# SGI-2022/Latent-Diffusion-Models-for-Shape-SDFs

Measured on AMD Instinct MI355X. Metric: SDF queries/sec on 256^3 grid (+ DDPM sample steps/sec), higher is better.
Workload: dtype bf16; 1 GPU; config4: decode B=64 shapes on a 256^3 grid on 1 rank (the whole grid is the one slab: no gather); batch=64, grid=256, latent_dim=256, decoder=DeepSDF 8x512 skip@4, parallelism=zslab1

## Files before the change

latent-diffusion-models-for-shape-sdfs_amd/csrc/decoder_fs.hip:

```cpp
#include "decoder_common.h"

namespace ldm {
namespace {
using namespace dec;

constexpr int kFsD = 4;

constexpr int kFsStep = 2048;
constexpr int kFsAct = 33 * 4 * 1024;
constexpr int kFsRed = 4 * 4 * 64 * 4;
constexpr int kFsWl = 512 * 4;
#ifndef FS_STAMP
#define FS_STAMP 0
#endif
constexpr int kFsStamp = FS_STAMP ? 128 * 8 : 0;
#ifndef FS_ABL
#define FS_ABL 0
#endif
static_assert(FS_ABL == 0 || FS_STAMP, "ablations are diagnostic builds");
constexpr int kFsLds = kFsAct + kFsRed + kFsWl + kFsStamp;
static_assert(kFsLds <= 160 * 1024, "LDS");

__host__ __device__ constexpr int fs_nparts(int S) { return S == 256 ? 15 : 16; }
__host__ __device__ constexpr int fs_nsteps(int S) { return S == 256 ? 384 : 448; }

template <typename T>
__global__ void fs_aux_pack_kernel(const float* __restrict__ beta, const float* __restrict__ wxyz,
                                   int B, T* __restrict__ aux) {
    const int id = blockIdx.x * blockDim.x + threadIdx.x;
    if (id >= B * 4 * 4 * 2 * 64) return;
    const int lane = id & 63;
    const int i = (id >> 6) & 1;
    const int slot = (id >> 7) & 3;
    const int w = (id >> 9) & 3;
    const int b = id >> 11;
    const int li = slot >> 1;
    const int p = slot & 1;
    float v[8] = {0, 0, 0, 0, 0, 0, 0, 0};
    if (lane < 32) {
        const int f = 128 * w + 64 * p + 32 * i + lane;
        const float* wx = wxyz + ((size_t)li * kHidden + f) * 3;
        const float bb = beta[((size_t)b * 2 + li) * kHidden + f];
        const float hi = Elem<T>::round(bb);
        v[0] = wx[0]; v[1] = wx[1]; v[2] = wx[2];
        v[3] = wx[0]; v[4] = wx[1]; v[5] = wx[2];
        v[6] = hi;    v[7] = bb - hi;
    }
    T* o = aux + (size_t)id * 8;
#pragma unroll
    for (int e = 0; e < 8; ++e) o[e] = (T)v[e];
}

struct FArgs {
    const uint8_t* stream;
    const uint8_t* aux;
    const float* w_last;
    const float* xyz;
    float* out;
    float b_last;
    int npts, tiles_per_shape, n_tiles;
    int N, k0;
    float vs, origin;
    const int32_t* bricks;
    const int32_t* count;
    int nb, nbt;
    GridDiv gd;
};

enum FsEpi { FE_NONE = 0, FE_LATE = 1, FE_EARLY = 2, FE_FIN0 = 3, FE_FIN1 = 4 };

struct FSrc {
    bool shape;
    uint32_t off;
    bool none = false;
};

struct FCtx {
    int lane, wave, h;
    uint32_t voff;
    char* smem;
    __amdgpu_buffer_rsrc_t rw;
    __amdgpu_buffer_rsrc_t ra;
    uint32_t s_beg, s_end;
    uint32_t s_iss;
    uint32_t baux_w;
    uint32_t aux_w;
    uint32_t aux_next;
    u32x4 auxn[2];
    u32x4 ring[kFsD][2];
    u32x4 b[4];
    float part[4];
    const f32x4* wlp;
    f32x4 wl[2][4];
    float* out;
    int npts, prev_shape, prev_local;
    float b_last;
    unsigned long long* st;
    int st_i;
    bool st_on;
    const int32_t* bricks;
    int N, nb, nbt;
};

__device__ __forceinline__ void stamp(FCtx& c) {
    if (FS_STAMP) {
        if (c.st_on && c.lane == 0 && c.st_i < 128) c.st[c.st_i] = __builtin_readcyclecounter();
        ++c.st_i;
    }
}

__device__ __forceinline__ u32x4 bld(__amdgpu_buffer_rsrc_t r, uint32_t voff, uint32_t soff) {
    return __builtin_bit_cast(u32x4, __builtin_amdgcn_raw_buffer_load_b128(r, voff, soff, 0));
}

__device__ __forceinline__ void load_aux(FCtx& c, FSrc s) {
    if (s.none) return;
    const __amdgpu_buffer_rsrc_t r = s.shape ? c.ra : c.rw;
    c.auxn[0] = bld(r, c.voff, s.off);
    c.auxn[1] = bld(r, c.voff + 1024u, s.off);
}

__device__ __forceinline__ uint32_t opaque(uint32_t v) {
    asm volatile("" : "+v"(v));
    return v;
}

__device__ __forceinline__ int opaque_s(int v) {
    asm volatile("" : "+s"(v));
    return v;
}

__device__ __forceinline__ char* lds_at(const FCtx& c, uint32_t off) {
    return c.smem + (opaque(c.voff) + off);
}
__device__ __forceinline__ char* lds_base(const FCtx& c, uint32_t off) {
    return c.smem + opaque(opaque(c.voff) + off);
}
__device__ __forceinline__ u32x4* act_wb(const FCtx& c, int late) {
    return reinterpret_cast<u32x4*>(lds_base(c, (uint32_t)(late + 4 * c.wave) * 4096u));
}
__device__ __forceinline__ u32x4* act_w(const FCtx& c, int late) {
    return reinterpret_cast<u32x4*>(lds_at(c, (uint32_t)(late + 4 * c.wave) * 4096u));
}
__device__ __forceinline__ const f32x4* wl_at(const FCtx& c, int p, int i) {
    const uint32_t h = opaque(c.voff) >> 9;
    return reinterpret_cast<const f32x4*>(
        c.smem + kFsAct + kFsRed + (((c.wave * 2 + p) * 2 + i) * 2) * 64 + h * 64);
}

__device__ __forceinline__ float* red_w(const FCtx& c) {
    return reinterpret_cast<float*>(c.smem + kFsAct + c.wave * 4 * 64 * 4 + (opaque(c.voff) >> 2));
}

__device__ __forceinline__ void fs_bar() {
    if (FS_ABL & 4) return;
    asm volatile("s_waitcnt lgkmcnt(0)\n\ts_barrier" ::: "memory");
}

__device__ __forceinline__ void read_b(FCtx& c, int pos) {
    const u32x4* p = reinterpret_cast<const u32x4*>(lds_at(c, pos * 4096));
#pragma unroll
    for (int n = 0; n < 4; ++n) c.b[n] = p[n * 64];
}

__device__ __forceinline__ void issue(FCtx& c, int r) {
    const uint32_t so = c.s_iss + (uint32_t)(r >> 1) * 2u * kFsStep;
    const uint32_t vo = c.voff + (uint32_t)(r & 1) * kFsStep;
    if (FS_ABL & 1) return;
    c.ring[r][0] = bld(c.rw, vo, so);
    c.ring[r][1] = bld(c.rw, vo + 1024u, so);
}

__device__ __forceinline__ uint32_t next_iss(const FCtx& c) {
    const uint32_t n = c.s_iss + 4u * kFsStep;
    return n == c.s_end ? c.s_beg : n;
}
__device__ __forceinline__ void next_group(FCtx& c) { c.s_iss = next_iss(c); }

__device__ __forceinline__ float relu_f(float x) {
    return __builtin_bit_cast(float, max(__builtin_bit_cast(int, x), 0));
}

__device__ __forceinline__ float acc_read(float a) {
    asm volatile("" : "+a"(a));
    return a;
}

__device__ __forceinline__ void fin1_unit(FCtx& c, const f32x16 (&accY)[2][4], int u) {
    const int t = u >> 1, s = u & 1;
    const int i = t >> 2, n = t & 3;
    const f32x4* w = wl_at(c, 1, i);
    float part = c.part[n];
#pragma unroll
    for (int q = 2 * s; q < 2 * s + 2; ++q) {
        const f32x4 wv = w[q];
#pragma unroll
        for (int e = 0; e < 4; ++e)
            part = fmaf(relu_f(acc_read(accY[i][n][4 * q + e])), wv[e], part);
    }
    c.part[n] = part;
}

template <typename T>
__device__ __forceinline__ void mfma_pair(f32x16 (&acc)[2][4], const u32x4& a0, const u32x4& a1,
                                          const u32x4& b, int n) {
    acc[0][n] = Elem<T>::mfma(a0, b, acc[0][n]);
    acc[1][n] = Elem<T>::mfma(a1, b, acc[1][n]);
}

template <typename T>
__device__ __forceinline__ void window_step(FCtx& c, f32x16 (&acc)[2][4],
                                            const f32x16 (&accY)[2][4], const u32x4& a0,
                                            const u32x4& a1, const u32x4* nb, int k, int r,
                                            u32x4* wbase) {
    uint32_t nxt = 0;
    if (k < 14) {
        const int t = k >> 1, s = k & 1;
        const int i = t >> 2, nn = t & 3;
        u32x4 f;
#pragma unroll
        for (int n = 0; n < 4; ++n) {
            unsigned w;
            if (r == 3 && n == 1) nxt = next_iss(c);
            const float e0 = accY[i][nn][8 * s + 2 * n], e1 = accY[i][nn][8 * s + 2 * n + 1];
            if (n < 3)
                Elem<T>::template pair_cvt1<false>(acc[0][n], acc[1][n], a0, a1, c.b[n], e0, e1,
                                                   w);
            else
                Elem<T>::template pair_cvt1<true>(acc[0][n], acc[1][n], a0, a1, c.b[n], e0, e1,
                                                  w);
            f[n] = w;
            c.b[n] = nb[n * 64];
            __builtin_amdgcn_sched_barrier(0);
        }
        issue(c, r);
        wbase[((2 * i + s) * 4 + nn) * 64] = f;
        if (r == 3) c.s_iss = nxt;
    } else {
        u32x4 f[2];
        const f32x16& y = accY[1][3];
#pragma unroll
        for (int p = 0; p < 4; ++p) {
            unsigned w0, w1;
            if (p < 3)
                Elem<T>::template pair_cvt2<false>(acc[0][p], acc[1][p], a0, a1, c.b[p], y[4 * p],
                                                   y[4 * p + 1], y[4 * p + 2], y[4 * p + 3], w0,
                                                   w1);
            else
                Elem<T>::template pair_cvt2<true>(acc[0][p], acc[1][p], a0, a1, c.b[p], y[4 * p],
                                                  y[4 * p + 1], y[4 * p + 2], y[4 * p + 3], w0,
                                                  w1);
            f[p >> 1][2 * (p & 1)] = w0;
            f[p >> 1][2 * (p & 1) + 1] = w1;
            c.b[p] = nb[p * 64];
            if (p == 1) wbase[(2 * 4 + 3) * 64] = f[0];
            __builtin_amdgcn_sched_barrier(0);
        }
        issue(c, r);
        wbase[(3 * 4 + 3) * 64] = f[1];
    }
    __builtin_amdgcn_sched_barrier(0);
}

template <typename T, int P>
__device__ __forceinline__ void window_step_fin(FCtx& c, f32x16 (&acc)[2][4],
                                                const f32x16 (&accY)[2][4], const u32x4& a0,
                                                const u32x4& a1, const u32x4* nb, int k, int r) {
    const int t = k >> 1, s = k & 1;
    const int i = t >> 2, nn = t & 3;
    const f32x16& y = accY[1][3];
    uint32_t nxt = 0;
    if (k == 0) {
        c.wlp = wl_at(c, P, 0);
#pragma unroll
        for (int q = 0; q < 4; ++q) c.wl[0][q] = c.wlp[q];
    }
#pragma unroll
    for (int n = 0; n < 4; ++n) {
        if (k < 14) {
            const int e = 8 * s + 2 * n;
            const float e0 = accY[i][nn][e], e1 = accY[i][nn][e + 1];
            const float w0 = c.wl[i][e >> 2][e & 3], w1 = c.wl[i][e >> 2][(e & 3) + 1];
            const int x = 2 * (k - 8) + n;
            if (k >= 8 && n < 2)
                Elem<T>::pair_fin3(acc[0][n], acc[1][n], a0, a1, c.b[n], e0, e1, w0, w1,
                                   c.part[nn], y[x], c.wl[1][x >> 2][x & 3], c.part[3]);
            else if (n < 3)
                Elem<T>::template pair_fin<false>(acc[0][n], acc[1][n], a0, a1, c.b[n], e0, e1,
                                                  w0, w1, c.part[nn]);
            else
                Elem<T>::template pair_fin<true>(acc[0][n], acc[1][n], a0, a1, c.b[n], e0, e1,
                                                 w0, w1, c.part[nn]);
        } else if (n < 2) {
            const int x = 12 + 2 * n;
            Elem<T>::template pair_fin<false>(acc[0][n], acc[1][n], a0, a1, c.b[n], y[x],
                                              y[x + 1], c.wl[1][3][x & 3],
                                              c.wl[1][3][(x & 3) + 1],
                                              c.part[3]);
        } else {
            mfma_pair<T>(acc, a0, a1, c.b[n], n);
        }
        if (r == 3 && n == 2) nxt = next_iss(c);
        c.b[n] = nb[n * 64];
        if (k == 6) c.wl[1][n] = c.wlp[8 + n];
        if (k == 14 && n == 2) {
            if (P == 0) {
#pragma unroll
                for (int m = 0; m < 4; ++m) asm volatile("" : "+v"(c.part[m]));
            } else {
                float* rw = red_w(c);
#pragma unroll
                for (int m = 0; m < 4; ++m) {
                    rw[m * 64] = c.part[m];
                    c.part[m] = 0.f;
                }
            }
        }
        __builtin_amdgcn_sched_barrier(0);
    }
    issue(c, r);
    if (r == 3) c.s_iss = nxt;
    __builtin_amdgcn_sched_barrier(0);
}

__device__ __forceinline__ void fin_store(const FCtx& c, int shape, int local) {
    const int lane = (int)(opaque(c.voff) >> 4);
    if (local < 0 || lane >= 32) return;
    const float* rr = reinterpret_cast<const float*>(
        c.smem + kFsAct + c.wave * 64 * 4 + (opaque(c.voff) >> 2));
    float s = 0.f;
#pragma unroll
    for (int w = 0; w < 4; ++w) s += rr[w * 4 * 64] + rr[w * 4 * 64 + 32];
    const int pt = local * kTilePoints + 32 * c.wave + lane;
    if (pt < c.npts) {
        const __amdgpu_buffer_rsrc_t ro = __builtin_amdgcn_make_buffer_rsrc(
            (void*)(c.out + (size_t)shape * c.npts), (short)0, 0x7ffffff0, 0x00020000);
        __builtin_amdgcn_raw_buffer_store_b32(__builtin_bit_cast(uint32_t, tanhf(s + c.b_last)),
                                              ro, (uint32_t)pt * 4u, 0, 2 );
    }
}

__device__ __forceinline__ int list_at(const int32_t* list, int i) {
    typedef const __attribute__((address_space(4))) int32_t* const_i32;
    return ((const_i32)(uintptr_t)list)[i];
}

__device__ __forceinline__ void brick_origin(int gid, int nb_, int& shape, int& i0, int& j0,
                                             int& k0) {
    const int nb = opaque_s(nb_);
    const int nb2 = nb * nb, nb3 = nb2 * nb;
    shape = gid / nb3;
    const int id = gid - shape * nb3;
    const int bz = id / nb2, r = id - bz * nb2;
    const int by = r / nb;
    i0 = 8 * (r - by * nb);
    j0 = 8 * by;
    k0 = 8 * bz;
}

__device__ __forceinline__ void fin_store_bricks(const FCtx& c, int tile) {
    const int lane = (int)(opaque(c.voff) >> 4);
    if (tile < 0 || lane >= 32) return;
    const float* rr = reinterpret_cast<const float*>(
        c.smem + kFsAct + c.wave * 64 * 4 + (opaque(c.voff) >> 2));
    float s = 0.f;
#pragma unroll
    for (int w = 0; w < 4; ++w) s += rr[w * 4 * 64] + rr[w * 4 * 64 + 32];
    const int gid = list_at(c.bricks, tile >> 2);
    LDM_DASSERT(gid >= 0 && gid < c.nbt);
    int shape, i0, j0, k0;
    brick_origin(gid, c.nb, shape, i0, j0, k0);
    const int idx = 128 * (tile & 3) + 32 * c.wave + lane;
    const int i = i0 + (idx & 7), j = j0 + ((idx >> 3) & 7);
    const int k = k0 + 2 * (tile & 3) + (c.wave >> 1);
    const int N = c.N;
    if ((unsigned)gid < (unsigned)c.nbt && i < N && j < N && k < N) {
        const __amdgpu_buffer_rsrc_t ro = __builtin_amdgcn_make_buffer_rsrc(
            (void*)(c.out + ((size_t)shape * N + k) * N * N), (short)0, 0x7ffffff0, 0x00020000);
        __builtin_amdgcn_raw_buffer_store_b32(__builtin_bit_cast(uint32_t, tanhf(s + c.b_last)),
                                              ro, (uint32_t)(j * N + i) * 4u, 0, 2 );
    }
}

template <int MODE>
__device__ __forceinline__ void fin_store_mode(const FCtx& c) {
    if (MODE == kModeBricks) fin_store_bricks(c, c.prev_local);
    else fin_store(c, c.prev_shape, c.prev_local);
}

template <typename T, int EK, int K0, int BAR, bool WIN = false>
__device__ __forceinline__ void group4(FCtx& c, f32x16 (&acc)[2][4], const f32x16 (&accY)[2][4],
                                       int p0, const char* gb = nullptr, u32x4* wb = nullptr,
                                       uint32_t* go = nullptr) {
    static_assert(WIN || EK == FE_NONE, "windows run through steps16e");
    constexpr int BP = 1;
    const bool carry = go != nullptr;
    const char* gbase = WIN ? gb : carry ? c.smem + *go + 4096 : lds_base(c, (p0 + 1) * 4096);
#pragma unroll
    for (int r = 0; r < 4; ++r) {
        const bool last = carry && r == 3;
        uint32_t nxt = 0;
        if (last) {
            nxt = next_iss(c);
            *go = opaque(*go + 4u * 4096u);
        }
        const u32x4* nb =
            reinterpret_cast<const u32x4*>(last ? c.smem + *go : gbase + r * 4096);
        const u32x4 a0 = c.ring[r][0], a1 = c.ring[r][1];
        const int k = K0 + r;
        if (r == BAR) {
#pragma unroll
            for (int n = 0; n < BP; ++n) mfma_pair<T>(acc, a0, a1, c.b[n], n);
            for (int n = 0; n < BP; ++n) {
                __builtin_amdgcn_sched_group_barrier(0x008, 2, 0);
            }
            __builtin_amdgcn_sched_barrier(0);
            fs_bar();
            __builtin_amdgcn_sched_barrier(0);
#pragma unroll
            for (int n = 0; n < BP; ++n) c.b[n] = nb[n * 64];
#pragma unroll
            for (int n = BP; n < 4; ++n) {
                mfma_pair<T>(acc, a0, a1, c.b[n], n);
                c.b[n] = nb[n * 64];
            }
            issue(c, r);
            for (int n = 0; n < BP; ++n) __builtin_amdgcn_sched_group_barrier(0x100, 1, 0);
            for (int n = BP; n < 4; ++n) {
                __builtin_amdgcn_sched_group_barrier(0x008, 2, 0);
                __builtin_amdgcn_sched_group_barrier(0x100, 1, 0);
            }
        } else if ((EK == FE_LATE || EK == FE_EARLY) && k < 15 && !(FS_ABL & 2)) {
            window_step<T>(c, acc, accY, a0, a1, nb, k, r, wb);
            if (r == 3) return;
            continue;
        } else if ((EK == FE_FIN0 || EK == FE_FIN1) && k < 15 && !(FS_ABL & 2)) {
            window_step_fin<T, EK == FE_FIN1>(c, acc, accY, a0, a1, nb, k, r);
            if (r == 3) return;
            continue;
        } else {
#pragma unroll
            for (int n = 0; n < 4; ++n) {
                mfma_pair<T>(acc, a0, a1, c.b[n], n);
                c.b[n] = nb[n * 64];
            }
            issue(c, r);
            if (last) c.s_iss = nxt;
#pragma unroll
            for (int n = 0; n < 4; ++n) {
                __builtin_amdgcn_sched_group_barrier(0x008, 2, 0);
                if (last && n == 0) {
                    __builtin_amdgcn_sched_group_barrier(0x004, 3, 0);
                    __builtin_amdgcn_sched_group_barrier(0x002, 1, 0);
                }
                __builtin_amdgcn_sched_group_barrier(0x100, 1, 0);
            }
        }
        __builtin_amdgcn_sched_group_barrier(0x020, 2, 0);
        __builtin_amdgcn_sched_barrier(0);
    }
    if (!carry) next_group(c);
}

template <typename T, int EK, bool BAR>
__device__ __forceinline__ void steps16e(FCtx& c, f32x16 (&acc)[2][4],
                                         const f32x16 (&accY)[2][4], int p0) {
    const char* gb = lds_base(c, (p0 + 1) * 4096);
    u32x4* wb = EK == FE_LATE ? act_wb(c, 16) : EK == FE_EARLY ? act_wb(c, 0) : nullptr;
    group4<T, EK, 0, -1, true>(c, acc, accY, p0, gb, wb);
    group4<T, EK, 4, -1, true>(c, acc, accY, p0 + 4, gb + 4 * 4096, wb);
    group4<T, EK, 8, -1, true>(c, acc, accY, p0 + 8, gb + 8 * 4096, wb);
    group4<T, EK, 12, BAR ? 3 : -1, true>(c, acc, accY, p0 + 12, gb + 12 * 4096, wb);
}

template <typename T>
__device__ __forceinline__ void steps_plain(FCtx& c, f32x16 (&acc)[2][4],
                                            const f32x16 (&accY)[2][4], int pos0, int j0, int j1) {
    if (j0 >= j1) return;
    uint32_t go = opaque(opaque(c.voff) + (uint32_t)(pos0 + j0) * 4096u);
#pragma unroll 1
    for (int j = j0; j < j1; j += 4)
        group4<T, FE_NONE, 0, -1>(c, acc, accY, pos0 + j, nullptr, nullptr, &go);
}

template <typename T, int EK, bool E16, int MODE = kModeGrid>
__device__ __forceinline__ void run_part(FCtx& c, f32x16 (&acc)[2][4], const f32x16 (&accY)[2][4],
                                         int nk, bool mid, bool endbar, FSrc naux, int pos0,
                                         bool bar0) {
    const f32x16 zero = {};
    const u32x4 a0 = c.auxn[0], a1 = c.auxn[1];
    if (bar0) {
#pragma unroll
        for (int n = 0; n < 4; ++n) {
            acc[0][n] = Elem<T>::mfma(a0, c.b[n], zero);
            acc[1][n] = Elem<T>::mfma(a1, c.b[n], zero);
        }
        load_aux(c, naux);
        fs_bar();
        read_b(c, pos0);
    } else {
        const u32x4* p = reinterpret_cast<const u32x4*>(lds_at(c, pos0 * 4096));
#pragma unroll
        for (int n = 0; n < 4; ++n) {
            acc[0][n] = Elem<T>::mfma(a0, c.b[n], zero);
            acc[1][n] = Elem<T>::mfma(a1, c.b[n], zero);
            c.b[n] = p[n * 64];
        }
        load_aux(c, naux);
#pragma unroll
        for (int n = 0; n < 4; ++n) {
            __builtin_amdgcn_sched_group_barrier(0x008, 2, 0);
            __builtin_amdgcn_sched_group_barrier(0x100, 1, 0);
        }
        __builtin_amdgcn_sched_group_barrier(0x020, 2, 0);
        __builtin_amdgcn_sched_barrier(0);
    }
    if (EK == FE_NONE) {
#pragma unroll
        for (int i = 0; i < 2; ++i)
#pragma unroll
            for (int n = 0; n < 4; ++n) asm volatile("" ::"a"(accY[i][n]));
    }
    stamp(c);
    if (!E16 && EK != FE_NONE) {
        if (mid || (endbar && nk == 16)) steps16e<T, EK, true>(c, acc, accY, pos0);
        else steps16e<T, EK, false>(c, acc, accY, pos0);
        if (EK == FE_FIN1) {
            stamp(c);
            fin_store_mode<MODE>(c);
        }
        stamp(c);
        if (endbar && nk == 32) {
            steps_plain<T>(c, acc, accY, pos0, 16, 28);
            group4<T, FE_NONE, 0, 3>(c, acc, accY, pos0 + 28);
        } else {
            steps_plain<T>(c, acc, accY, pos0, 16, nk);
        }
    } else if (E16) {
        static_assert(!E16 || EK == FE_EARLY, "E16 parts convert part 0 of their own layer");
        steps_plain<T>(c, acc, accY, pos0, 0, 12);
        group4<T, FE_NONE, 0, 3>(c, acc, accY, pos0 + 12);
        stamp(c);
        if (endbar) steps16e<T, EK, true>(c, acc, accY, pos0 + 16);
        else steps16e<T, EK, false>(c, acc, accY, pos0 + 16);
    } else {
        steps_plain<T>(c, acc, accY, pos0, 0, nk < 16 ? nk : 16);
        stamp(c);
        steps_plain<T>(c, acc, accY, pos0, 16, nk);
    }
    stamp(c);
}

template <typename T>
__device__ __forceinline__ void acc_to_lds(FCtx& c, const f32x16 (&acc)[2][4]) {
    u32x4* p = act_w(c, 16);
#pragma unroll
    for (int i = 0; i < 2; ++i)
#pragma unroll
        for (int n = 0; n < 4; ++n) {
            u32x4 f0, f1;
            acc_to_frags<T>(acc[i][n], f0, f1);
            p[(2 * i * 4 + n) * 64] = f0;
            p[((2 * i + 1) * 4 + n) * 64] = f1;
        }
}

template <typename T, bool LATE>
__device__ __forceinline__ void layer0_part(FCtx& c, FSrc naux) {
    const u32x4 a[2] = {c.auxn[0], c.auxn[1]};
    u32x4* p = act_w(c, LATE ? 16 : 0);
    f32x16 t[2];
    t[0] = Elem<T>::mfma_v(a[0], c.b[0]);
#pragma unroll
    for (int q = 0; q < 8; ++q) {
        const int i = q & 1, n = q >> 1;
        if (q < 7) t[(q + 1) & 1] = Elem<T>::mfma_v(a[(q + 1) & 1], c.b[(q + 1) >> 1]);
        if (q == 0) {
            asm volatile("s_nop 10" : "+v"(t[0]));
            load_aux(c, naux);
            stamp(c);
        }
        __builtin_amdgcn_sched_barrier(0);
        u32x4 f0, f1;
        acc_to_frags<T>(t[q & 1], f0, f1);
        p[(2 * i * 4 + n) * 64] = f0;
        p[((2 * i + 1) * 4 + n) * 64] = f1;
        __builtin_amdgcn_sched_barrier(0);
    }
    stamp(c);
}

template <typename T, int S, int MODE>
__global__ __launch_bounds__(256, 1) void dec_fs_kernel(FArgs a) {
    __shared__ __attribute__((aligned(16))) char smem[kFsLds];
    FCtx c;
    c.lane = threadIdx.x & 63;
    c.wave = __builtin_amdgcn_readfirstlane(threadIdx.x >> 6);
    c.h = c.lane >> 5;
    c.voff = (uint32_t)c.lane * 16u;
    c.smem = smem;
    c.out = a.out;
    c.npts = a.npts;
    c.b_last = a.b_last;
    c.prev_shape = 0;
    c.prev_local = -1;
    c.st = reinterpret_cast<unsigned long long*>(smem + kFsAct + kFsRed + kFsWl);
    c.st_i = 0;
    c.st_on = false;
    float* wl = reinterpret_cast<float*>(smem + kFsAct + kFsRed);

    for (int i = threadIdx.x; i < 512; i += 256) wl[i] = a.w_last[i];
    __syncthreads();
    const int n_tiles = MODE == kModeBricks ? 4 * min(max(a.count[0], 0), a.nbt) : a.n_tiles;
    if (MODE == kModeBricks) {
        c.bricks = a.bricks;
        c.N = a.N;
        c.nb = a.nb;
        c.nbt = a.nbt;
    }
    if ((int)blockIdx.x >= n_tiles) return;

    constexpr int NST = fs_nsteps(S);
    constexpr int NP = fs_nparts(S);
    constexpr uint32_t kFlags = 0x00020000u;
    c.rw = __builtin_amdgcn_make_buffer_rsrc((void*)a.stream, (short)0, 0x7ffffff0, kFlags);
    c.ra = __builtin_amdgcn_make_buffer_rsrc((void*)a.aux, (short)0, 0x7ffffff0, kFlags);
    c.s_beg = (uint32_t)c.wave * NST * kFsStep;
    c.s_end = c.s_beg + NST * kFsStep;
    c.s_iss = c.s_beg;
    c.baux_w = (uint32_t)(4 * NST + c.wave * NP) * kFsStep;
    auto brick_of = [&](int tile) -> int {
        return min(max(list_at(a.bricks, tile >> 2), 0), a.nbt - 1);
    };
    auto shape_aux = [&](int tile) -> uint32_t {
        if (MODE == kModeBricks) {
            const int nb = opaque_s(a.nb);
            return ((uint32_t)(brick_of(tile) / (nb * nb * nb)) * 4u + (uint32_t)c.wave) * 4u *
                   kFsStep;
        }
        return ((uint32_t)(tile / a.tiles_per_shape) * 4u + (uint32_t)c.wave) * 4u * kFsStep;
    };
    auto bias = [&](int pi) -> FSrc { return FSrc{false, c.baux_w + (uint32_t)pi * kFsStep}; };
    auto shp = [&](int slot) -> FSrc { return FSrc{true, c.aux_w + (uint32_t)slot * kFsStep}; };
    c.aux_w = shape_aux(blockIdx.x);
#pragma unroll
    for (int r = 0; r < kFsD; ++r) issue(c, r);
    next_group(c);

    f32x16 accA[2][4], accB[2][4];
#pragma unroll
    for (int i = 0; i < 2; ++i)
#pragma unroll
        for (int n = 0; n < 4; ++n) accB[i][n] = f32x16{};
#pragma unroll
    for (int n = 0; n < 4; ++n) c.part[n] = 0.f;
#pragma unroll 1
    for (int tile = blockIdx.x; tile < n_tiles; tile += gridDim.x) {
        int shape, local, bi0 = 0, bj0 = 0, bk0 = 0;
        if (MODE == kModeBricks) {
            brick_origin(brick_of(tile), a.nb, shape, bi0, bj0, bk0);
            local = tile;
        } else {
            shape = tile / a.tiles_per_shape;
            local = tile - shape * a.tiles_per_shape;
        }
        {
            const int nt = tile + (int)gridDim.x;
            c.aux_next = nt < n_tiles ? shape_aux(nt) : c.aux_w;
        }
        c.st_on = FS_STAMP && c.wave == 0 && tile == (int)blockIdx.x + (int)gridDim.x;
        c.st_i = 0;
        stamp(c);
        load_aux(c, shp(0));
        const uint32_t lv = opaque(c.voff);
        const bool hi = lv >= 512u;
        const uint32_t p0 = (uint32_t)local * kTilePoints;
        uint32_t ti = 0, tj = 0, tk = 0;
        if (MODE == kModeGrid) {
            grid_first(p0, (uint32_t)a.N, a.gd, ti, tj, tk);
            tk += (uint32_t)a.k0;
        }
        const float* row = nullptr;
        if (MODE == kModePoints) {
            row = a.xyz + (size_t)shape * a.npts * 3;
            asm volatile("" : "+s"(row));
        }
#pragma unroll
        for (int n = 0; n < 4; ++n) {
            int pt = local * kTilePoints + 32 * n + (int)((lv >> 4) & 31u);
            if (pt >= a.npts) pt = a.npts - 1;
            float x, y, z;
            if (MODE == kModeBricks) {
                const int idx = 128 * (tile & 3) + 32 * n + (int)((lv >> 4) & 31u);
                const int m = a.N - 1;
                x = grid_axis(min(bi0 + (idx & 7), m), a.vs, a.origin);
                y = grid_axis(min(bj0 + ((idx >> 3) & 7), m), a.vs, a.origin);
                z = grid_axis(min(bk0 + (idx >> 6), m), a.vs, a.origin);
            } else if (MODE == kModePoints) {
                const float* qq = row + (size_t)pt * 3;
                x = qq[0];
                y = qq[1];
                z = qq[2];
            } else {
                const uint32_t off =
                    grid_tail_off(p0, 32u * n + ((lv >> 4) & 31u), (uint32_t)a.npts);
                uint32_t vi, vj, vk;
                grid_voxel(ti, tj, tk, off, (uint32_t)a.N, a.gd.m, vi, vj, vk);
                x = grid_axis((int)vi, a.vs, a.origin);
                y = grid_axis((int)vj, a.vs, a.origin);
                z = grid_axis((int)vk, a.vs, a.origin);
            }
            const float xh = Elem<T>::round(x), yh = Elem<T>::round(y), zh = Elem<T>::round(z);
            u32x4 f;
            f[0] = hi ? 0u : Elem<T>::pack(xh, yh);
            f[1] = hi ? 0u : Elem<T>::pack(zh, x - xh);
            f[2] = hi ? 0u : Elem<T>::pack(y - yh, z - zh);
            f[3] = hi ? 0u : Elem<T>::pack(1.f, 1.f);
            reinterpret_cast<u32x4*>(lds_at(c, 32u * 4096u))[n * 64] = f;
        }
        read_b(c, 32);

        layer0_part<T, false>(c, shp(1));
        layer0_part<T, true>(c, bias(2));

        int pi = 2;
        run_part<T, FE_FIN1, false, MODE>(c, accA, accB, 32, true, false, bias(pi + 1), 0, true);
        run_part<T, FE_EARLY, true>(c, accB, accA, 32, true, true, bias(pi + 2), 0, false);
        pi += 2;
        constexpr int L2P = S == 256 ? 3 : 4;
#pragma unroll 1
        for (int l = 2; l < L2P; ++l, pi += 2) {
            const FSrc nx = (S == 512 && l == 3) ? shp(2) : bias(pi + 2);
            run_part<T, FE_LATE, false>(c, accA, accB, 32, true, false, bias(pi + 1), 0,
                                                false);
            run_part<T, FE_EARLY, true>(c, accB, accA, 32, true, true, nx, 0, false);
        }
        if (S == 256) {
            run_part<T, FE_LATE, false>(c, accA, accB, 32, true, false, shp(2), 0,
                                                false);
            fs_bar();
            acc_to_lds<T>(c, accA);
            stamp(c);
            run_part<T, FE_NONE, false>(c, accA, accB, 16, false, false, shp(3), 16, true);
            run_part<T, FE_EARLY, false>(c, accB, accA, 16, false, true, bias(pi + 3),
                                                  16, false);
            pi += 3;
        } else {
            run_part<T, FE_LATE, false>(c, accA, accB, 32, true, false, shp(3), 0,
                                                false);
            run_part<T, FE_EARLY, true>(c, accB, accA, 32, true, true, bias(pi + 2), 0,
                                                 false);
            pi += 2;
        }
#pragma unroll 1
        for (int l = 5; l < 7; ++l, pi += 2) {
            run_part<T, FE_LATE, false>(c, accA, accB, 32, true, false, bias(pi + 1), 0,
                                                 false);
            run_part<T, FE_EARLY, true>(c, accB, accA, 32, true, true, bias(pi + 2), 0,
                                                 false);
        }
        run_part<T, FE_LATE, false>(c, accA, accB, 32, true, false, bias(pi + 1), 0,
                                             false);
        run_part<T, FE_FIN0, false>(c, accB, accA, 32, false, true, FSrc{true, 0, true},
                                             0, false);
        c.prev_shape = shape;
        c.prev_local = local;
        c.aux_w = c.aux_next;
    }
#pragma unroll
    for (int u = 0; u < 16; ++u) fin1_unit(c, accB, u);
    {
        float* rw = red_w(c);
#pragma unroll
        for (int n = 0; n < 4; ++n) rw[n * 64] = c.part[n];
    }
    fs_bar();
    fin_store_mode<MODE>(c);
    asm volatile("s_waitcnt vmcnt(0)" ::: "memory");
    if (FS_STAMP && c.wave == 0) {
        __builtin_amdgcn_s_waitcnt(0);
        for (int k = c.lane; k < 128; k += 64)
            reinterpret_cast<unsigned long long*>(a.out)[(size_t)blockIdx.x * 128 + k] = c.st[k];
    }
}

template <typename T, int S>
void launch_fs(const FArgs& a, bool points, hipStream_t s, int grid) {
    if (points)
        hipLaunchKernelGGL((dec_fs_kernel<T, S, kModePoints>), dim3(grid), dim3(256), 0, s, a);
    else
        hipLaunchKernelGGL((dec_fs_kernel<T, S, kModeGrid>), dim3(grid), dim3(256), 0, s, a);
}

template <typename T, int S>
void launch_fs_bricks(const FArgs& a, hipStream_t s, int grid) {
    hipLaunchKernelGGL((dec_fs_kernel<T, S, kModeBricks>), dim3(grid), dim3(256), 0, s, a);
}

}

size_t decoder_fs_aux_bytes(int B) { return (size_t)B * 4 * 4 * kFsStep; }

int decoder_fs_n_stages(int skip_width) { return fs_nsteps(skip_width == 253 ? 256 : 512); }

int decoder_fs_fwd(const ldm_decoder_t* w, const float* beta, const float* xyz, int B, int npts,
                   int N, int k0, float vs, float origin, float* out, void* ws, size_t ws_bytes,
                   hipStream_t s, int num_cus, const int32_t* bricks, const int32_t* count,
                   int n_bricks) {
    const int S = w->skip_width == 253 ? 256 : 512;
    LDM_REQUIRE(w->n_stages == fs_nsteps(S), LDM_EINVAL, "split layout: n_stages %d != %d",
                w->n_stages, fs_nsteps(S));
    LDM_REQUIRE(ws != nullptr && ws_bytes >= decoder_fs_aux_bytes(B) && LDM_ALIGNED(ws, 16),
                LDM_ENOSPC, "workspace too small: need %zu bytes, got %zu",
                decoder_fs_aux_bytes(B), ws_bytes);
    LDM_REQUIRE((size_t)B * 4 * 4 * kFsStep < 0x7ffffff0u, LDM_EINVAL,
                "split layout: %d shapes exceed the aux buffer range", B);
    {
        const int n = B * 4 * 4 * 2 * 64;
        if (w->dtype == LDM_BF16)
            hipLaunchKernelGGL(fs_aux_pack_kernel<__bf16>, dim3((n + 255) / 256), dim3(256), 0, s,
                               beta, w->wxyz, B, (__bf16*)ws);
        else
            hipLaunchKernelGGL(fs_aux_pack_kernel<_Float16>, dim3((n + 255) / 256), dim3(256), 0,
                               s, beta, w->wxyz, B, (_Float16*)ws);
        if (int e = launch_status("fs_aux_pack")) return e;
    }
    FArgs a;
    a.stream = (const uint8_t*)w->weights;
    a.aux = (const uint8_t*)ws;
    a.w_last = w->w_last;
    a.xyz = xyz;
    a.out = out;
    a.b_last = w->b_last;
    a.npts = npts;
    a.tiles_per_shape = (npts + kTilePoints - 1) / kTilePoints;
    a.n_tiles = B * a.tiles_per_shape;
    a.bricks = bricks;
    a.count = count;
    a.nb = (N + 7) / 8;
    a.nbt = n_bricks;
    const int mode = bricks ? kModeBricks : xyz ? kModePoints : kModeGrid;
    if (mode == kModeBricks) a.n_tiles = 4 * n_bricks;
    a.N = N;
    a.k0 = k0;
    a.vs = vs;
    a.origin = origin;
    a.gd = mode == kModeGrid ? grid_div(N) : GridDiv{0, 0, 0};
    const int grid = a.n_tiles < num_cus ? a.n_tiles : num_cus;
    if (mode != kModeBricks) {
        const bool points = mode == kModePoints;
        if (w->dtype == LDM_BF16) {
            if (S == 256) launch_fs<__bf16, 256>(a, points, s, grid);
            else launch_fs<__bf16, 512>(a, points, s, grid);
        } else {
            if (S == 256) launch_fs<_Float16, 256>(a, points, s, grid);
            else launch_fs<_Float16, 512>(a, points, s, grid);
        }
    } else if (w->dtype == LDM_BF16) {
        if (S == 256) launch_fs_bricks<__bf16, 256>(a, s, grid);
        else launch_fs_bricks<__bf16, 512>(a, s, grid);
    } else {
        if (S == 256) launch_fs_bricks<_Float16, 256>(a, s, grid);
        else launch_fs_bricks<_Float16, 512>(a, s, grid);
    }
    return launch_status("ldm_decoder_fwd(split)");
}

}
```

Before: 493.4 million queries/s.

## Precompute per-part bias images in LDS and seed accumulators from them

For the even-numbered layer parts, the kernel now computes the per-shape bias contribution once at kernel start with an MFMA against a ones vector and stores it as an accumulator image in LDS. Parts that used a bias aux MFMA at step 0 instead read this image during the previous part's barrier step and start their accumulation from it. This drops the per-tile aux load and bias MFMA for those parts. In exchange it uses extra LDS, adds register pressure for the image, and changes the scheduling hints around the barrier.

```diff
diff --git a/latent-diffusion-models-for-shape-sdfs_amd/csrc/decoder_fs.hip b/latent-diffusion-models-for-shape-sdfs_amd/csrc/decoder_fs.hip
--- a/latent-diffusion-models-for-shape-sdfs_amd/csrc/decoder_fs.hip
+++ b/latent-diffusion-models-for-shape-sdfs_amd/csrc/decoder_fs.hip
@@ -10,6 +10,9 @@
 constexpr int kFsAct = 33 * 4 * 1024;
 constexpr int kFsRed = 4 * 4 * 64 * 4;
 constexpr int kFsWl = 512 * 4;
+constexpr int kFsImgRow = 2 * 2 * 16 * 4;
+constexpr int kFsImg = 4 * 16 * kFsImgRow;
+constexpr int kFsImgOff = kFsAct + kFsRed + kFsWl;
 #ifndef FS_STAMP
 #define FS_STAMP 0
 #endif
@@ -18,11 +21,17 @@
 #define FS_ABL 0
 #endif
 static_assert(FS_ABL == 0 || FS_STAMP, "ablations are diagnostic builds");
-constexpr int kFsLds = kFsAct + kFsRed + kFsWl + kFsStamp;
+constexpr int kFsLds = kFsAct + kFsRed + kFsWl + kFsImg + kFsStamp;
 static_assert(kFsLds <= 160 * 1024, "LDS");
 
 __host__ __device__ constexpr int fs_nparts(int S) { return S == 256 ? 15 : 16; }
 __host__ __device__ constexpr int fs_nsteps(int S) { return S == 256 ? 384 : 448; }
+static_assert(fs_nparts(512) * 4 * kFsImgRow <= kFsImg, "bias images");
+__host__ __device__ constexpr int fs_nimg(int S) { return S == 256 ? 4 : 5; }
+__host__ __device__ constexpr int fs_img_part(int S, int k) {
+    return S == 256 ? (k == 0 ? 3 : k == 1 ? 5 : k == 2 ? 10 : 12)
+                    : (k == 0 ? 3 : k == 1 ? 5 : k == 2 ? 7 : k == 3 ? 11 : 13);
+}
 
 template <typename T>
 __global__ void fs_aux_pack_kernel(const float* __restrict__ beta, const float* __restrict__ wxyz,
@@ -148,6 +157,20 @@
         c.smem + kFsAct + kFsRed + (((c.wave * 2 + p) * 2 + i) * 2) * 64 + h * 64);
 }
 
+__device__ __forceinline__ const f32x4* img_at(const FCtx& c, int pi) {
+    const uint32_t h = opaque(c.voff) >> 9;
+    return reinterpret_cast<const f32x4*>(
+        c.smem + kFsImgOff + (uint32_t)(c.wave * 16 + pi) * kFsImgRow + h * 64);
+}
+__device__ __forceinline__ void img_read(f32x16 (&img)[2], const f32x4* ip) {
+#pragma unroll
+    for (int i = 0; i < 2; ++i) {
+        const f32x4 t0 = ip[8 * i], t1 = ip[8 * i + 1], t2 = ip[8 * i + 2], t3 = ip[8 * i + 3];
+        img[i] = f32x16{t0[0], t0[1], t0[2], t0[3], t1[0], t1[1], t1[2], t1[3],
+                        t2[0], t2[1], t2[2], t2[3], t3[0], t3[1], t3[2], t3[3]};
+    }
+}
+
 __device__ __forceinline__ float* red_w(const FCtx& c) {
     return reinterpret_cast<float*>(c.smem + kFsAct + c.wave * 4 * 64 * 4 + (opaque(c.voff) >> 2));
 }
@@ -388,11 +411,16 @@
     else fin_store(c, c.prev_shape, c.prev_local);
 }
 
-template <typename T, int EK, int K0, int BAR, bool WIN = false>
+enum FsImg { kImgNone = 0, kImgStart = 1, kImgLoad = 2 };
+template <typename T, int EK, int K0, int BAR, bool WIN = false, int IMG = kImgNone>
 __device__ __forceinline__ void group4(FCtx& c, f32x16 (&acc)[2][4], const f32x16 (&accY)[2][4],
                                        int p0, const char* gb = nullptr, u32x4* wb = nullptr,
-                                       uint32_t* go = nullptr) {
+                                       uint32_t* go = nullptr, f32x16 (*img)[2] = nullptr,
+                                       int ipi = 0, FSrc naux = FSrc{false, 0, true},
+                                       int lastpos = -1) {
     static_assert(WIN || EK == FE_NONE, "windows run through steps16e");
+    static_assert(IMG != kImgLoad || BAR >= 0, "the image is read in the barrier step");
+    static_assert(IMG != kImgStart || (BAR != 0 && !WIN), "step 0 of a plain group");
     constexpr int BP = 1;
     const bool carry = go != nullptr;
     const char* gbase = WIN ? gb : carry ? c.smem + *go + 4096 : lds_base(c, (p0 + 1) * 4096);
@@ -404,8 +432,9 @@
             nxt = next_iss(c);
             *go = opaque(*go + 4u * 4096u);
         }
-        const u32x4* nb =
-            reinterpret_cast<const u32x4*>(last ? c.smem + *go : gbase + r * 4096);
+        const u32x4* nb = reinterpret_cast<const u32x4*>(
+            last ? c.smem + *go
+                 : (r == 3 && lastpos >= 0) ? lds_at(c, lastpos * 4096) : gbase + r * 4096);
         const u32x4 a0 = c.ring[r][0], a1 = c.ring[r][1];
         const int k = K0 + r;
         if (r == BAR) {
@@ -419,16 +448,35 @@
             __builtin_amdgcn_sched_barrier(0);
 #pragma unroll
             for (int n = 0; n < BP; ++n) c.b[n] = nb[n * 64];
+            if (IMG == kImgLoad) {
+                const f32x4* ip = img_at(c, ipi);
+                img_read(*img, ip);
+            }
 #pragma unroll
             for (int n = BP; n < 4; ++n) {
                 mfma_pair<T>(acc, a0, a1, c.b[n], n);
                 c.b[n] = nb[n * 64];
             }
             issue(c, r);
-            for (int n = 0; n < BP; ++n) __builtin_amdgcn_sched_group_barrier(0x100, 1, 0);
-            for (int n = BP; n < 4; ++n) {
+            if (IMG == kImgLoad) {
+                static_assert(IMG != kImgLoad || BP == 1, "the image reads' places");
+                __builtin_amdgcn_sched_group_barrier(0x100, 3, 0);
+                __builtin_amdgcn_sched_group_barrier(0x008, 1, 0);
+                __builtin_amdgcn_sched_group_barrier(0x100, 2, 0);
+                __builtin_amdgcn_sched_group_barrier(0x008, 1, 0);
+                __builtin_amdgcn_sched_group_barrier(0x100, 2, 0);
+                __builtin_amdgcn_sched_group_barrier(0x008, 1, 0);
+                __builtin_amdgcn_sched_group_barrier(0x100, 3, 0);
+                __builtin_amdgcn_sched_group_barrier(0x008, 1, 0);
+                __builtin_amdgcn_sched_group_barrier(0x100, 1, 0);
                 __builtin_amdgcn_sched_group_barrier(0x008, 2, 0);
                 __builtin_amdgcn_sched_group_barrier(0x100, 1, 0);
+            } else {
+                for (int n = 0; n < BP; ++n) __builtin_amdgcn_sched_group_barrier(0x100, 1, 0);
+                for (int n = BP; n < 4; ++n) {
+                    __builtin_amdgcn_sched_group_barrier(0x008, 2, 0);
+                    __builtin_amdgcn_sched_group_barrier(0x100, 1, 0);
+                }
             }
         } else if ((EK == FE_LATE || EK == FE_EARLY) && k < 15 && !(FS_ABL & 2)) {
             window_step<T>(c, acc, accY, a0, a1, nb, k, r, wb);
@@ -439,9 +487,16 @@
             if (r == 3) return;
             continue;
         } else {
+            const bool start = IMG == kImgStart && r == 0;
 #pragma unroll
             for (int n = 0; n < 4; ++n) {
-                mfma_pair<T>(acc, a0, a1, c.b[n], n);
+                if (start) {
+                    acc[0][n] = Elem<T>::mfma(a0, c.b[n], (*img)[0]);
+                    acc[1][n] = Elem<T>::mfma(a1, c.b[n], (*img)[1]);
+                } else {
+                    mfma_pair<T>(acc, a0, a1, c.b[n], n);
+                }
+                if (start && n == 0) load_aux(c, naux);
                 c.b[n] = nb[n * 64];
             }
             issue(c, r);
@@ -453,6 +508,8 @@
                     __builtin_amdgcn_sched_group_barrier(0x004, 3, 0);
                     __builtin_amdgcn_sched_group_barrier(0x002, 1, 0);
                 }
+                if (start && n == 0 && !naux.none)
+                    __builtin_amdgcn_sched_group_barrier(0x020, 2, 0);
                 __builtin_amdgcn_sched_group_barrier(0x100, 1, 0);
             }
         }
@@ -462,15 +519,17 @@
     if (!carry) next_group(c);
 }
 
-template <typename T, int EK, bool BAR>
+template <typename T, int EK, bool BAR, int IMG = kImgNone>
 __device__ __forceinline__ void steps16e(FCtx& c, f32x16 (&acc)[2][4],
-                                         const f32x16 (&accY)[2][4], int p0) {
+                                         const f32x16 (&accY)[2][4], int p0,
+                                         f32x16 (*img)[2] = nullptr, int ipi = 0) {
     const char* gb = lds_base(c, (p0 + 1) * 4096);
     u32x4* wb = EK == FE_LATE ? act_wb(c, 16) : EK == FE_EARLY ? act_wb(c, 0) : nullptr;
     group4<T, EK, 0, -1, true>(c, acc, accY, p0, gb, wb);
     group4<T, EK, 4, -1, true>(c, acc, accY, p0 + 4, gb + 4 * 4096, wb);
     group4<T, EK, 8, -1, true>(c, acc, accY, p0 + 8, gb + 8 * 4096, wb);
-    group4<T, EK, 12, BAR ? 3 : -1, true>(c, acc, accY, p0 + 12, gb + 12 * 4096, wb);
+    group4<T, EK, 12, BAR ? 3 : -1, true, IMG>(c, acc, accY, p0 + 12, gb + 12 * 4096, wb, nullptr,
+                                               img, ipi);
 }
 
 template <typename T>
@@ -483,13 +542,16 @@
         group4<T, FE_NONE, 0, -1>(c, acc, accY, pos0 + j, nullptr, nullptr, &go);
 }
 
-template <typename T, int EK, bool E16, int MODE = kModeGrid>
+template <typename T, int EK, bool E16, int MODE = kModeGrid, int IMG = kImgNone>
 __device__ __forceinline__ void run_part(FCtx& c, f32x16 (&acc)[2][4], const f32x16 (&accY)[2][4],
                                          int nk, bool mid, bool endbar, FSrc naux, int pos0,
-                                         bool bar0) {
+                                         bool bar0, f32x16 (&img)[2], int ipi = 0) {
+    static_assert(IMG != kImgStart || E16, "image parts start with plain steps");
+    static_assert(IMG != kImgLoad || (!E16 && EK != FE_NONE), "the image is read in a window");
     const f32x16 zero = {};
     const u32x4 a0 = c.auxn[0], a1 = c.auxn[1];
-    if (bar0) {
+    if (IMG == kImgStart) {
+    } else if (bar0) {
 #pragma unroll
         for (int n = 0; n < 4; ++n) {
             acc[0][n] = Elem<T>::mfma(a0, c.b[n], zero);
@@ -523,7 +585,8 @@
     }
     stamp(c);
     if (!E16 && EK != FE_NONE) {
-        if (mid || (endbar && nk == 16)) steps16e<T, EK, true>(c, acc, accY, pos0);
+        if (IMG == kImgLoad) steps16e<T, EK, true, kImgLoad>(c, acc, accY, pos0, &img, ipi);
+        else if (mid || (endbar && nk == 16)) steps16e<T, EK, true>(c, acc, accY, pos0);
         else steps16e<T, EK, false>(c, acc, accY, pos0);
         if (EK == FE_FIN1) {
             stamp(c);
@@ -533,12 +596,22 @@
         if (endbar && nk == 32) {
             steps_plain<T>(c, acc, accY, pos0, 16, 28);
             group4<T, FE_NONE, 0, 3>(c, acc, accY, pos0 + 28);
+        } else if (IMG == kImgLoad) {
+            steps_plain<T>(c, acc, accY, pos0, 16, 28);
+            group4<T, FE_NONE, 0, -1>(c, acc, accY, pos0 + 28, nullptr, nullptr, nullptr, nullptr,
+                                      0, FSrc{false, 0, true}, 0);
         } else {
             steps_plain<T>(c, acc, accY, pos0, 16, nk);
         }
     } else if (E16) {
         static_assert(!E16 || EK == FE_EARLY, "E16 parts convert part 0 of their own layer");
-        steps_plain<T>(c, acc, accY, pos0, 0, 12);
+        if (IMG == kImgStart) {
+            group4<T, FE_NONE, 0, -1, false, kImgStart>(c, acc, accY, pos0, nullptr, nullptr,
+                                                        nullptr, &img, 0, naux);
+            steps_plain<T>(c, acc, accY, pos0, 4, 12);
+        } else {
+            steps_plain<T>(c, acc, accY, pos0, 0, 12);
+        }
         group4<T, FE_NONE, 0, 3>(c, acc, accY, pos0 + 12);
         stamp(c);
         if (endbar) steps16e<T, EK, true>(c, acc, accY, pos0 + 16);
@@ -549,6 +622,13 @@
         steps_plain<T>(c, acc, accY, pos0, 16, nk);
     }
     stamp(c);
+}
+
+__device__ __forceinline__ void fs_pin_set(f32x16 (&s)[2][4]) {
+#pragma unroll
+    for (int i = 0; i < 2; ++i)
+#pragma unroll
+        for (int n = 0; n < 4; ++n) asm volatile("" : "+a"(s[i][n]));
 }
 
 template <typename T>
@@ -604,7 +684,7 @@
     c.b_last = a.b_last;
     c.prev_shape = 0;
     c.prev_local = -1;
-    c.st = reinterpret_cast<unsigned long long*>(smem + kFsAct + kFsRed + kFsWl);
+    c.st = reinterpret_cast<unsigned long long*>(smem + kFsImgOff + kFsImg);
     c.st_i = 0;
     c.st_on = false;
     float* wl = reinterpret_cast<float*>(smem + kFsAct + kFsRed);
@@ -647,7 +727,34 @@
     for (int r = 0; r < kFsD; ++r) issue(c, r);
     next_group(c);
 
+    {
+        constexpr int NI = fs_nimg(S);
+        u32x4 fa[NI][2];
+#pragma unroll
+        for (int k = 0; k < NI; ++k) {
+            const uint32_t so = c.baux_w + (uint32_t)fs_img_part(S, k) * kFsStep;
+            fa[k][0] = bld(c.rw, c.voff, so);
+            fa[k][1] = bld(c.rw, c.voff + 1024u, so);
+        }
+        const u32x4 one = {0u, 0u, 0u, c.lane < 32 ? Elem<T>::pack(1.f, 1.f) : 0u};
+#pragma unroll
+        for (int k = 0; k < NI; ++k)
+#pragma unroll
+            for (int i = 0; i < 2; ++i) {
+                const f32x16 d = Elem<T>::mfma(fa[k][i], one, f32x16{});
+                f32x4* o = reinterpret_cast<f32x4*>(
+                    smem + kFsImgOff + (c.wave * 16 + fs_img_part(S, k)) * kFsImgRow + i * 128 +
+                    c.h * 64);
+                if ((c.lane & 31) == 0) {
+#pragma unroll
+                    for (int q = 0; q < 4; ++q)
+                        o[q] = f32x4{d[4 * q], d[4 * q + 1], d[4 * q + 2], d[4 * q + 3]};
+                }
+            }
+    }
+
     f32x16 accA[2][4], accB[2][4];
+    f32x16 img[2];
 #pragma unroll
     for (int i = 0; i < 2; ++i)
 #pragma unroll
@@ -724,45 +831,51 @@
         layer0_part<T, true>(c, bias(2));
 
         int pi = 2;
-        run_part<T, FE_FIN1, false, MODE>(c, accA, accB, 32, true, false, bias(pi + 1), 0, true);
-        run_part<T, FE_EARLY, true>(c, accB, accA, 32, true, true, bias(pi + 2), 0, false);
+        const FSrc none = FSrc{false, 0, true};
+        run_part<T, FE_FIN1, false, MODE, kImgLoad>(c, accA, accB, 32, true, false, none, 0, true,
+                                                    img, pi + 1);
+        run_part<T, FE_EARLY, true, kModeGrid, kImgStart>(c, accB, accA, 32, true, true,
+                                                          bias(pi + 2), 0, false, img);
         pi += 2;
         constexpr int L2P = S == 256 ? 3 : 4;
 #pragma unroll 1
         for (int l = 2; l < L2P; ++l, pi += 2) {
             const FSrc nx = (S == 512 && l == 3) ? shp(2) : bias(pi + 2);
-            run_part<T, FE_LATE, false>(c, accA, accB, 32, true, false, bias(pi + 1), 0,
-                                                false);
-            run_part<T, FE_EARLY, true>(c, accB, accA, 32, true, true, nx, 0, false);
+            run_part<T, FE_LATE, false, kModeGrid, kImgLoad>(c, accA, accB, 32, true, false, none,
+                                                             0, false, img, pi + 1);
+            run_part<T, FE_EARLY, true, kModeGrid, kImgStart>(c, accB, accA, 32, true, true, nx, 0,
+                                                              false, img);
         }
         if (S == 256) {
             run_part<T, FE_LATE, false>(c, accA, accB, 32, true, false, shp(2), 0,
-                                                false);
+                                                false, img);
             fs_bar();
             acc_to_lds<T>(c, accA);
             stamp(c);
-            run_part<T, FE_NONE, false>(c, accA, accB, 16, false, false, shp(3), 16, true);
+            run_part<T, FE_NONE, false>(c, accA, accB, 16, false, false, shp(3), 16, true, img);
             run_part<T, FE_EARLY, false>(c, accB, accA, 16, false, true, bias(pi + 3),
-                                                  16, false);
+                                                  16, false, img);
             pi += 3;
         } else {
             run_part<T, FE_LATE, false>(c, accA, accB, 32, true, false, shp(3), 0,
-                                                false);
+                                                false, img);
             run_part<T, FE_EARLY, true>(c, accB, accA, 32, true, true, bias(pi + 2), 0,
-                                                 false);
+                                                 false, img);
             pi += 2;
         }
+        fs_pin_set(accB);
 #pragma unroll 1
         for (int l = 5; l < 7; ++l, pi += 2) {
-            run_part<T, FE_LATE, false>(c, accA, accB, 32, true, false, bias(pi + 1), 0,
-                                                 false);
-            run_part<T, FE_EARLY, true>(c, accB, accA, 32, true, true, bias(pi + 2), 0,
-                                                 false);
-        }
+            run_part<T, FE_LATE, false, kModeGrid, kImgLoad>(c, accA, accB, 32, true, false, none,
+                                                             0, false, img, pi + 1);
+            run_part<T, FE_EARLY, true, kModeGrid, kImgStart>(c, accB, accA, 32, true, true,
+                                                              bias(pi + 2), 0, false, img);
+        }
+        fs_pin_set(accB);
         run_part<T, FE_LATE, false>(c, accA, accB, 32, true, false, bias(pi + 1), 0,
-                                             false);
+                                             false, img);
         run_part<T, FE_FIN0, false>(c, accB, accA, 32, false, true, FSrc{true, 0, true},
-                                             0, false);
+                                             0, false, img);
         c.prev_shape = shape;
         c.prev_local = local;
         c.aux_w = c.aux_next;
```

Result: no change. 493.3 million queries/s (-0.0%).
